# travelingspaceman/LowThrustOpt

Hardware: NVIDIA B200
Metric: segment-propagations/s (fp64 state+STM) (higher is better)
Workload: dtype f64

## Files before the change

lowthrustopt_b200/csrc/lto_capi.cu:

```cuda
#include "../../include/lto_b200.h"
#include "lto_internal.h"
#include "lto_handle.h"
#include <cstdio>
#include <cstring>
#include <cstdarg>
#include <algorithm>
#include <cstdlib>
#include <cmath>
#include <thread>
#include <vector>

using namespace lto;

static char g_err[512] = "";

int lto_fail(lto_handle* h, int code, const char* fmt, ...) {
    char buf[512];
    va_list ap; va_start(ap, fmt); vsnprintf(buf, sizeof buf, fmt, ap); va_end(ap);
    snprintf(g_err, sizeof g_err, "%s", buf);
    if (h) snprintf(h->err, sizeof h->err, "%s", buf);
    return code;
}

int lto_ensure(lto_handle* h, void** p, size_t* cap, size_t need) {
// ... 134 lines not shown
}
double lto_last_kernel_ms(const lto_handle* h) {
    if (!h) return 0.0;
    double ms = h->last_ms;
    for (int i = 0; i < h->n_child; ++i) ms = std::max(ms, h->child[i]->last_ms);
    return ms;
}
int lto_n_devices(const lto_handle* h) { return h ? (h->n_child > 0 ? h->n_child : 1) : 0; }
void* lto_stream(lto_handle* h) { return (h && h->n_child == 0) ? (void*)h->s_compute : nullptr; }
int lto_sync(lto_handle* h) {
    LTO_NVTX();
    if (!h) return fail(nullptr, LTO_ERR_ARG, "null handle");
    for (int i = 0; i < h->n_child; ++i) { int rc = lto_sync(h->child[i]); if (rc) return fail(h, rc, "%s", h->child[i]->err); }
    if (h->n_child > 0) return LTO_SUCCESS;
    CK(h, cudaSetDevice(h->device));
    CK(h, cudaStreamSynchronize(h->s_compute));
    return LTO_SUCCESS;
}

}

static int make_direct(lto_handle* h, const lto_direct_params* p, int nstate, int nsteps, DirectArgs* a) {
    if (!p) return fail(h, LTO_ERR_ARG, "null params");
    if (nstate != 6 && nstate != 7) return fail(h, LTO_ERR_ARG, "nstate must be 6 or 7 (got %d)", nstate);
    if (p->mode != LTO_FIXED && p->mode != LTO_ADAPTIVE) return fail(h, LTO_ERR_ARG, "bad mode %d", p->mode);
    if (p->mode == LTO_FIXED && nsteps < 2) return fail(h, LTO_ERR_ARG, "nsteps must be >= 2 (got %d)", nsteps);
    const double g0 = p->g0 > 0 ? p->g0 : 9.81;
    a->c.mu = p->MU; a->c.m1 = 1.0 - p->MU;
    a->c.kthr = p->TU * p->TU / p->DU / 1e3;
    a->c.cmdot = p->TU / (p->Isp * g0);
    a->c.default_mass = p->default_mass > 0 ? p->default_mass : 1000.0;
    a->cfg.mode = p->mode; a->cfg.nsteps = nsteps; a->cfg.tol = p->tol > 0 ? p->tol : 1e-13;
    a->cfg.err_norm = p->err_norm; a->cfg.max_attempts = p->max_attempts > 0 ? p->max_attempts : 100000;
    return 0;
}
static int make_indirect(lto_handle* h, const lto_indirect_params* p, int ndim, bool sens, IndirectArgs* a) {
    if (!p) return fail(h, LTO_ERR_ARG, "null params");
    if (ndim != 12 && ndim != 14) return fail(h, LTO_ERR_ARG, "ndim must be 12 or 14 (got %d)", ndim);
    if (!(p->p == 0.0 || p->p >= 1.0)) return fail(h, LTO_ERR_ARG, "Invalid value of p!");
    const double g0 = p->g0 > 0 ? p->g0 : 9.81;
    a->c.mu = p->MU; a->c.m1 = 1.0 - p->MU;
    a->c.kthr = p->TU * p->TU / p->DU / 1e3;
    a->c.thrustLimit = p->thrustLimit; a->c.mass = p->mass; a->c.omega = p->time_direction;
    a->c.p = p->p; a->c.rho = p->rho;
    a->c.cm = p->TU / (a->c.kthr * (p->Isp > 0 ? p->Isp : 2000.0) * g0);
    a->cfg.atol = p->abstol > 0 ? p->abstol : 1e-13; a->cfg.rtol = p->reltol > 0 ? p->reltol : 1e-13;
    a->cfg.controller = p->controller; a->cfg.err_norm = sens ? p->err_norm : 0;
    a->cfg.max_attempts = p->max_attempts > 0 ? p->max_attempts : 100000;
    return 0;
}

static int dispatch_direct(lto_handle* h, const DirectArgs& a, int nstate, int kernel) {
    int nl = 0;
    cudaError_t e = cudaErrorNotSupported;
    if (kernel != LTO_KERNEL_GENERIC) e = launch_direct_fast(a, nstate, h->s_compute, &nl);
    if (e == cudaErrorNotSupported) {
        if (kernel == LTO_KERNEL_FAST) return fail(h, LTO_ERR_ARG, "LTO_KERNEL_FAST does not cover this configuration");
        e = launch_direct_generic(a, nstate, h->s_compute, &nl);
    }
    h->launches += nl;
    if (e != cudaSuccess) return fail(h, LTO_ERR_CUDA, "direct kernel launch: %s", cudaGetErrorString(e));
    return 0;
}
static int dispatch_indirect(lto_handle* h, const IndirectArgs& a, int ndim, int kernel, cudaStream_t st = nullptr) {
    int nl = 0;
    if (!st) st = h->s_compute;
// ... 538 lines not shown
```

lowthrustopt_b200/csrc/lto_direct_cw.cu:

```cuda
#include "lto_internal.h"
#include "lto_cw_common.cuh"
#include <algorithm>

namespace lto {

namespace cw {

constexpr int NTILE = 2;
constexpr int NSLOT = 2;
constexpr int XW0 = 2;

template <int NS>
struct Cfg {
    static constexpr int NCOL = NS + 3;
    static constexpr int NW = NTILE + NCOL;
    static constexpr int NTHREADS = 32 * NW;
    static constexpr int SVAL = (NS == 7) ? 10 : 6;
    static constexpr int OFF_H = 13 * SVAL;
    static constexpr int OFF_BM = OFF_H + 1;
    static constexpr int STEP_DOUBLES = OFF_BM + ((NS == 7) ? 3 : 0);
    static constexpr size_t REC_BYTES = (size_t)NTILE * NSLOT * STEP_DOUBLES * 32 * sizeof(double);
    static constexpr int NV = 2 * (NS + 3);
    static constexpr size_t OUT_TILE_BYTES = (size_t)16 * NS * NV * sizeof(double);
    static constexpr size_t OUT_BYTES = (size_t)NTILE * OUT_TILE_BYTES;
    static constexpr size_t BAR_OFF = REC_BYTES + OUT_BYTES;
    static constexpr size_t FLAG_OFF = BAR_OFF + (size_t)NTILE * NSLOT * 2 * sizeof(unsigned long long);
    static constexpr size_t SMEM = FLAG_OFF + (size_t)NTILE * NSLOT * sizeof(int);
};

using namespace cwc;

template <int NS, bool PUB = true>
__device__ __forceinline__ double x_step(double (&r)[3], double (&v)[3], double& m, const double (&u)[3], double omega,
                                         double mdot, double h, const EPConst& c, double* __restrict__ rec, double& maxErr) {
    constexpr int SVAL = Cfg<NS>::SVAL;
    const double h2 = h * h;
    const double w2 = 2.0 * omega;
    const double kom6 = c.kthr / c.default_mass;
    double a[13][3];
    double ev[3] = {0.0, 0.0, 0.0}, ea[3] = {0.0, 0.0, 0.0};
    if (PUB) rec[Cfg<NS>::OFF_H * 32] = h;
#pragma unroll
    for (int j = 0; j < 13; ++j) {
        double R[3], V[3];
#pragma unroll
        for (int q = 0; q < 3; ++q) {
            double accv = 0.0, accr = 0.0;
#pragma unroll
            for (int l = 0; l < j; ++l) {
                if (lto_tab::Bf(j, l) != 0.0) accv = fma(lto_tab::Bf(j, l), a[l][q], accv);
                if (lto_tab::Gf(j, l) != 0.0) accr = fma(lto_tab::Gf(j, l), a[l][q], accr);
            }
            V[q] = (j == 0) ? v[q] : fma(h, accv, v[q]);
            R[q] = (j == 0) ? r[q] : fma(h2, accr, fma(h * lto_tab::Cf(j), v[q], r[q]));
        }
        const double dx1 = R[0] + c.mu, dx2 = dx1 - 1.0;
        const double yz = fma(R[1], R[1], R[2] * R[2]);
        const double i1 = fast_rsqrt(fma(dx1, dx1, yz));
        const double i2 = fast_rsqrt(fma(dx2, dx2, yz));
        const double i1s = i1 * i1, i2s = i2 * i2;
        const double a31 = c.m1 * i1s * i1, a32 = c.mu * i2s * i2;
        const double gg1 = 1.0 - (a31 + a32);
        double kom = kom6, im = 0.0;
        if (NS == 7) { im = fast_rcp(fma(h * lto_tab::Cf(j), mdot, m)); kom = c.kthr * im; }
        a[j][0] = fma(u[0], kom, fma(-a31, dx1, fma(-a32, dx2, fma(w2, V[1], R[0]))));
        a[j][1] = fma(u[1], kom, fma(gg1, R[1], -w2 * V[0]));
        a[j][2] = fma(u[2], kom, (gg1 - 1.0) * R[2]);
        if (PUB && j != 10) {
            const double a51 = 3.0 * i1s * a31, a52 = 3.0 * i2s * a32;
            const double s5 = a51 + a52;
            const double p1 = a51 * dx1, p2 = a52 * dx2;
            const double t = p1 + p2;
            const double s5y = s5 * R[1];
            double* w = rec + j * SVAL * 32;
            w[0 * 32] = fma(p1, dx1, fma(p2, dx2, gg1));
            w[1 * 32] = fma(s5y, R[1], gg1);
            w[2 * 32] = fma(s5 * R[2], R[2], gg1 - 1.0);
            w[3 * 32] = t * R[1];
            w[4 * 32] = t * R[2];
            w[5 * 32] = s5y * R[2];
            if (NS == 7) {
                w[6 * 32] = kom;
                const double k2 = -kom * im;
#pragma unroll
                for (int q = 0; q < 3; ++q) w[(7 + q) * 32] = k2 * u[q];
            }
        }
        if (lto_tab::PSIf(j) != 0.0) {
#pragma unroll
            for (int q = 0; q < 3; ++q) { ev[q] = fma(lto_tab::PSIf(j), V[q], ev[q]); ea[q] = fma(lto_tab::PSIf(j), a[j][q], ea[q]); }
        }
    }
    double delta = 0.0;
#pragma unroll
    for (int q = 0; q < 3; ++q) {
        double sv = 0.0, sr = 0.0;
#pragma unroll
        for (int l = 0; l < 13; ++l) {
            if (lto_tab::CHIf(l) != 0.0) sv = fma(lto_tab::CHIf(l), a[l][q], sv);
            if (lto_tab::CHIBf(l) != 0.0) sr = fma(lto_tab::CHIBf(l), a[l][q], sr);
        }
        r[q] = fma(h2, sr, fma(h, v[q], r[q]));
        v[q] = fma(h, sv, v[q]);
        delta = fmax(delta, fmax(fabs(ev[q]), fabs(ea[q])));
    }
    if (NS == 7) m = fma(h, mdot, m);
    delta *= fabs(h * lto_tab::ERRC);
    maxErr = fmax(maxErr, delta);
    return delta;
}

template <int NS>
__device__ __forceinline__ void col_step(double (&sr)[3], double (&sv)[3], double& sm, double bm, const double (&ec)[3],
                                         double omega, double kom6, const double* __restrict__ rec) {
    constexpr int SVAL = Cfg<NS>::SVAL;
    constexpr bool MASS = (NS == 7);
    const double h = rec[Cfg<NS>::OFF_H * 32];
    const double h2 = h * h;
    const double w2 = 2.0 * omega;
    double a[13][3];
#pragma unroll
    for (int j = 0; j < 13; ++j) {
        if (j == 10) continue;
        double R[3], V[3];
#pragma unroll
        for (int q = 0; q < 3; ++q) {
            double accv = 0.0, accr = 0.0;
#pragma unroll
            for (int l = 0; l < j; ++l) {
                if (lto_tab::Bf(j, l) != 0.0) accv = fma(lto_tab::Bf(j, l), a[l][q], accv);
                if (lto_tab::Gf(j, l) != 0.0) accr = fma(lto_tab::Gf(j, l), a[l][q], accr);
            }
            V[q] = (j == 0) ? sv[q] : fma(h, accv, sv[q]);
            R[q] = (j == 0) ? sr[q] : fma(h2, accr, fma(h * lto_tab::Cf(j), sv[q], sr[q]));
        }
        const double* w = rec + j * SVAL * 32;
        double U[6];
#pragma unroll
        for (int q = 0; q < 6; ++q) U[q] = w[q * 32];
        const double kom = MASS ? w[6 * 32] : kom6;
        double acc[3];
        acc[0] = fma(ec[0], kom, w2 * V[1]);
        acc[1] = fma(ec[1], kom, -w2 * V[0]);
        acc[2] = ec[2] * kom;
        if (MASS) {
            const double smj = fma(h * lto_tab::Cf(j), bm, sm);
#pragma unroll
            for (int q = 0; q < 3; ++q) acc[q] = fma(w[(7 + q) * 32], smj, acc[q]);
        }
        sym3_mul_acc(U, R, acc);
#pragma unroll
        for (int q = 0; q < 3; ++q) a[j][q] = acc[q];
    }
#pragma unroll
    for (int q = 0; q < 3; ++q) {
        double dv = 0.0, dr = 0.0;
#pragma unroll
        for (int l = 0; l < 13; ++l) {
            if (lto_tab::CHIf(l) != 0.0) dv = fma(lto_tab::CHIf(l), a[l][q], dv);
            if (lto_tab::CHIBf(l) != 0.0) dr = fma(lto_tab::CHIBf(l), a[l][q], dr);
        }
        sr[q] = fma(h2, dr, fma(h, sv[q], sr[q]));
        sv[q] = fma(h, dv, sv[q]);
    }
    if (MASS) sm = fma(h, bm, sm);
}

struct ColState { double sr[3], sv[3], sm, bm; };

template <int NS>
__device__ __forceinline__ void col_init(ColState& c, int col) {
#pragma unroll
    for (int q = 0; q < 3; ++q) { c.sr[q] = (col == q) ? 1.0 : 0.0; c.sv[q] = (col == q + 3) ? 1.0 : 0.0; }
    c.sm = (NS == 7 && col == 6) ? 1.0 : 0.0;
    c.bm = 0.0;
}

template <int NS>
__device__ __forceinline__ void col_store(double* __restrict__ stage, const ColState& c, int col, int lane) {
    constexpr int NV = 2 * (NS + 3);
    const int back = lane & 1, gc = col - NS;
    const int ocol = (gc >= 0) ? (2 * NS + (back ? 3 : 0) + gc) : ((back ? NS : 0) + col);
    double* J = stage + (lane >> 1) * (NS * NV) + ocol * NS;
    const double rj = (col >= 3 && col < 6) ? -1.0 : 1.0;
    const double sp = back ? -rj : 1.0;
    const double sq = back ? rj : 1.0;
    J[0] = sp * c.sr[0]; J[1] = sp * c.sr[1]; J[2] = sp * c.sr[2];
    J[3] = sq * c.sv[0]; J[4] = sq * c.sv[1]; J[5] = sq * c.sv[2];
    if (NS == 7) J[6] = sp * c.sm;
}

template <int NS>
__device__ __forceinline__ void column_warp(const DirectArgs& a, long long n_tiles, int col, int lane, double* recs, double* outs, unsigned bars) {
    typedef Cfg<NS> C;
    const int nstep = a.cfg.nsteps - 1;
    const double omega = (lane & 1) ? -1.0 : 1.0;
    const double kom6 = a.c.kthr / a.c.default_mass;
    const int gc = col - NS;
    const double ec[3] = {gc == 0 ? 1.0 : 0.0, gc == 1 ? 1.0 : 0.0, gc == 2 ? 1.0 : 0.0};
    ColState cs[NTILE];
    unsigned g = 0;
    for (long long pair = blockIdx.x; pair * NTILE < n_tiles; pair += gridDim.x) {
#pragma unroll
        for (int t = 0; t < NTILE; ++t) col_init<NS>(cs[t], col);
        for (int k = 0; k < nstep; ++k, ++g) {
            const unsigned slot = g & (NSLOT - 1), par = (g / NSLOT) & 1;
#ifndef LTO_K1_NO_PACE
            asm volatile("bar.sync 3, %0;" ::"n"(32 * C::NCOL) : "memory");
#endif
#pragma unroll
            for (int t = 0; t < NTILE; ++t) {
                const double* rec = recs + (size_t)(t * NSLOT + slot) * C::STEP_DOUBLES * 32 + lane;
                const unsigned full = bars + (unsigned)((t * NSLOT + slot) * 16), empty = full + 8;
                mbar_wait(full, par);
                if (NS == 7 && k == 0 && gc >= 0) cs[t].bm = rec[(C::OFF_BM + gc) * 32];
                col_step<NS>(cs[t].sr, cs[t].sv, cs[t].sm, cs[t].bm, ec, omega, kom6, rec);
                mbar_arrive(empty);
                if (k == nstep - 1) {
                    const long long tile = pair * NTILE + t;
                    const long long seg0 = tile * 16;
                    double* stage = outs + (size_t)t * (C::OUT_TILE_BYTES / sizeof(double));
                    const bool leader = (col == 0 && lane == 0);
                    if (leader) bulk_store_wait_read_but<NTILE - 1>();
                    asm volatile("bar.sync 2, %0;" ::"n"(32 * C::NCOL) : "memory");
                    col_store<NS>(stage, cs[t], col, lane);
                    fence_proxy_async();
                    asm volatile("bar.sync 2, %0;" ::"n"(32 * C::NCOL) : "memory");
                    if (leader && seg0 < a.n_seg) {
                        const long long nseg = (a.n_seg - seg0 < 16) ? (a.n_seg - seg0) : 16;
                        bulk_store(a.jac + seg0 * (long long)(NS * C::NV), smem_u32(stage), (unsigned)(nseg * NS * C::NV * sizeof(double)));
                    }
                }
            }
        }
    }
    if (col == 0 && lane == 0) bulk_store_wait_all();
}

template <int NS>
__device__ __forceinline__ void state_warp(const DirectArgs& a, long long n_tiles, int t, int lane, double* recs, unsigned bars) {
    typedef Cfg<NS> C;
    const int nsteps = a.cfg.nsteps, nstep = nsteps - 1;
    const int back = lane & 1;
    const double omega = back ? -1.0 : 1.0;
    double r[3], v[3], m = a.c.default_mass, u[3], bm[3] = {0.0, 0.0, 0.0}, mdot = 0.0, t0 = 0.0, t1 = 1.0, maxErr = 0.0;
    unsigned g = 0;
    for (long long pair = blockIdx.x; pair * NTILE < n_tiles; pair += gridDim.x) {
        const long long seg = (pair * NTILE + t) * 16 + (lane >> 1);
        {
            const long long sc = seg < a.n_seg ? seg : a.n_seg - 1;
            const long long ia = lto_node_a(sc, a.npt);
            const double* X = (back ? a.Xb : a.Xa) + ia * NS;
            const double* U = (back ? a.ub : a.ua) + ia * 3;
            r[0] = X[0]; r[1] = X[1]; r[2] = X[2];
            v[0] = X[3]; v[1] = X[4]; v[2] = X[5];
            if (back) { v[0] = -v[0]; v[1] = -v[1]; v[2] = -v[2]; }
            if (NS == 7) m = X[6];
            u[0] = U[0]; u[1] = U[1]; u[2] = U[2];
            const double ta = a.ta[ia], tb = a.tb[ia];
            t0 = ta; t1 = ta + (tb - ta) / 2.0;
            const double un = sqrt(fma(u[0], u[0], fma(u[1], u[1], u[2] * u[2])));
            mdot = -omega * un * a.c.cmdot;
            if (NS == 7) {
#pragma unroll
                for (int q = 0; q < 3; ++q) {
                    const double uh = (un > 0.0) ? u[q] / un : 1.0;
                    bm[q] = -omega * a.c.cmdot * uh;
                }
            }
            maxErr = 0.0;
        }
        for (int k = 0; k < nstep; ++k, ++g) {
            const unsigned slot = g & (NSLOT - 1), use = g / NSLOT;
            double* rec = recs + (size_t)(t * NSLOT + slot) * C::STEP_DOUBLES * 32 + lane;
            const unsigned full = bars + (unsigned)((t * NSLOT + slot) * 16), empty = full + 8;
            if (use > 0) mbar_wait(empty, (use - 1) & 1);
            const double h = linrange_at(t0, t1, nsteps, k + 1) - linrange_at(t0, t1, nsteps, k);
            if (NS == 7) {
#pragma unroll
                for (int q = 0; q < 3; ++q) rec[(C::OFF_BM + q) * 32] = bm[q];
            }
            x_step<NS>(r, v, m, u, omega, mdot, h, a.c, rec, maxErr);
            mbar_arrive(full);
        }
        const unsigned fullmask = 0xffffffffu;
        double xe[NS];
        xe[0] = r[0]; xe[1] = r[1]; xe[2] = r[2];
        xe[3] = back ? -v[0] : v[0]; xe[4] = back ? -v[1] : v[1]; xe[5] = back ? -v[2] : v[2];
        if (NS == 7) xe[6] = m;
        bool bad = false;
#pragma unroll
        for (int q = 0; q < NS; ++q) {
            const double other = __shfl_xor_sync(fullmask, xe[q], 1);
            const double d = xe[q] - other;
            bad |= !(d == d);
            if (!back && seg < a.n_seg) a.defect[seg * NS + q] = d;
        }
        const double me_o = __shfl_xor_sync(fullmask, maxErr, 1);
        if (!back && seg < a.n_seg) {
            if (a.errors) a.errors[seg] = fmax(maxErr, me_o);
            if (a.status) a.status[seg] = bad ? LTO_ST_NAN : LTO_OK;
        }
    }
}


template <int NS>
__device__ __forceinline__ void state_warp_adapt(const DirectArgs& a, long long n_tiles, int t, int lane, double* recs, unsigned bars, volatile int* lastf) {
    typedef Cfg<NS> C;
    const int back = lane & 1;
    const double omega = back ? -1.0 : 1.0;
    const unsigned fullmask = 0xffffffffu;
    double r[3], v[3], m = a.c.default_mass, u[3], bm[3] = {0.0, 0.0, 0.0}, mdot = 0.0, dummy = 0.0;
    unsigned g = 0;
    for (long long pair = blockIdx.x; pair * NTILE < n_tiles; pair += gridDim.x) {
        const long long seg = (pair * NTILE + t) * 16 + (lane >> 1);
        const long long sc = seg < a.n_seg ? seg : a.n_seg - 1;
        const long long ia = lto_node_a(sc, a.npt);
        const double* X = (back ? a.Xb : a.Xa) + ia * NS;
        const double* U = (back ? a.ub : a.ua) + ia * 3;
        r[0] = X[0]; r[1] = X[1]; r[2] = X[2];
        v[0] = X[3]; v[1] = X[4]; v[2] = X[5];
        if (back) { v[0] = -v[0]; v[1] = -v[1]; v[2] = -v[2]; }
        if (NS == 7) m = X[6];
        u[0] = U[0]; u[1] = U[1]; u[2] = U[2];
        const double ta = a.ta[ia], tb = a.tb[ia];
        const double t0 = ta, tfinal = ta + (tb - ta) / 2.0;
        const double un = sqrt(fma(u[0], u[0], fma(u[1], u[1], u[2] * u[2])));
        mdot = -omega * un * a.c.cmdot;
        if (NS == 7) {
#pragma unroll
            for (int q = 0; q < 3; ++q) { const double uh = (un > 0.0) ? u[q] / un : 1.0; bm[q] = -omega * a.c.cmdot * uh; }
        }
        const double hmax = (tfinal - t0) / 2.5, hmin = (tfinal - t0) / 1e7;
        double tt = t0, h = (tfinal - t0) / 50.0;
        int status = 0, nt = 0;
        bool done = !((tt < tfinal) && (h >= hmin));
        while (true) {
            const unsigned slot = g & (NSLOT - 1), use = g / NSLOT;
            double* rec = recs + (size_t)(t * NSLOT + slot) * C::STEP_DOUBLES * 32 + lane;
            const unsigned full = bars + (unsigned)((t * NSLOT + slot) * 16), empty = full + 8;
            if (use > 0) mbar_wait(empty, (use - 1) & 1);
            if (NS == 7) {
#pragma unroll
                for (int q = 0; q < 3; ++q) rec[(C::OFF_BM + q) * 32] = bm[q];
            }
            bool pending = !done;
            if (done) {
#pragma unroll
                for (int j = 0; j < 13 * C::SVAL; ++j) rec[j * 32] = 0.0;
                rec[C::OFF_H * 32] = 0.0;
            }
            while (__any_sync(fullmask, pending)) {
                if (pending) {
                    if (tt + h > tfinal) h = tfinal - tt;
                    if (nt >= a.cfg.max_attempts) { status = LTO_ST_MAXSTEPS; done = true; pending = false; }
                }
                if (pending) {
                    ++nt;
                    double r2[3] = {r[0], r[1], r[2]}, v2[3] = {v[0], v[1], v[2]}, m2 = m;
                    const double xn = fmax(fmax(fmax(fabs(r[0]), fabs(r[1])), fmax(fabs(r[2]), fabs(v[0]))), fmax(fmax(fabs(v[1]), fabs(v[2])), NS == 7 ? fabs(m) : 0.0));
                    double delta = x_step<NS>(r2, v2, m2, u, omega, mdot, h, a.c, rec, dummy);
                    if (!(delta == delta)) { status = LTO_ST_NAN; done = true; pending = false; }
                    else {
                        const double tau = a.cfg.tol * fmax(xn, 1.0);
                        if (delta <= tau) {
                            tt += h;
                            r[0] = r2[0]; r[1] = r2[1]; r[2] = r2[2]; v[0] = v2[0]; v[1] = v2[1]; v[2] = v2[2]; m = m2;
                            pending = false;
                        }
                        if (delta == 0.0) delta = 1e-16;
                        h = fmin(hmax, 0.8 * h * pow(tau / delta, 0.125));
                        if (!((tt < tfinal) && (h >= hmin))) { done = true; if (pending) { status = LTO_ST_HMIN; pending = false; } }
                    }
                }
            }
            if (status != 0) {
#pragma unroll
                for (int j = 0; j < 13 * C::SVAL; ++j) rec[j * 32] = 0.0;
                rec[C::OFF_H * 32] = 0.0;
            }
            const bool all_done = __all_sync(fullmask, done);
            if (lane == 0) lastf[t * NSLOT + slot] = all_done ? 1 : 0;
            mbar_arrive(full);
            ++g;
            if (all_done) break;
        }
        if (status == 0 && tt < tfinal) status = LTO_ST_HMIN;
        double xe[NS];
        xe[0] = r[0]; xe[1] = r[1]; xe[2] = r[2];
        xe[3] = back ? -v[0] : v[0]; xe[4] = back ? -v[1] : v[1]; xe[5] = back ? -v[2] : v[2];
        if (NS == 7) xe[6] = m;
        bool bad = false;
#pragma unroll
        for (int q = 0; q < NS; ++q) {
            const double other = __shfl_xor_sync(fullmask, xe[q], 1);
            const double d = xe[q] - other;
            bad |= !(d == d);
            if (!back && seg < a.n_seg) a.defect[seg * NS + q] = d;
        }
        const int st_o = __shfl_xor_sync(fullmask, status, 1);
        if (!back && seg < a.n_seg) {
            if (a.errors) a.errors[seg] = 0.0;
            if (a.status) a.status[seg] = status ? status : (st_o ? st_o : (bad ? LTO_ST_NAN : LTO_OK));
        }
    }
}

template <int NS>
__device__ __forceinline__ void column_warp_adapt(const DirectArgs& a, long long n_tiles, int col, int lane, double* recs, double* outs, unsigned bars,
                                                  volatile int* lastf) {
    typedef Cfg<NS> C;
    const double omega = (lane & 1) ? -1.0 : 1.0;
    const double kom6 = a.c.kthr / a.c.default_mass;
    const int gc = col - NS;
    const double ec[3] = {gc == 0 ? 1.0 : 0.0, gc == 1 ? 1.0 : 0.0, gc == 2 ? 1.0 : 0.0};
    ColState cs[NTILE];
    unsigned g[NTILE];
#pragma unroll
    for (int t = 0; t < NTILE; ++t) g[t] = 0;
    for (long long pair = blockIdx.x; pair * NTILE < n_tiles; pair += gridDim.x) {
#pragma unroll
        for (int t = 0; t < NTILE; ++t) col_init<NS>(cs[t], col);
        unsigned alive = (1u << NTILE) - 1u, first = alive;
        while (alive) {
#ifndef LTO_K1_NO_PACE
            asm volatile("bar.sync 3, %0;" ::"n"(32 * C::NCOL) : "memory");
#endif
#pragma unroll
            for (int t = 0; t < NTILE; ++t) {
                if (!(alive & (1u << t))) continue;
                const unsigned slot = g[t] & (NSLOT - 1), par = (g[t] / NSLOT) & 1;
                const double* rec = recs + (size_t)(t * NSLOT + slot) * C::STEP_DOUBLES * 32 + lane;
                const unsigned full = bars + (unsigned)((t * NSLOT + slot) * 16), empty = full + 8;
                mbar_wait(full, par);
                if (NS == 7 && (first & (1u << t)) && gc >= 0) cs[t].bm = rec[(C::OFF_BM + gc) * 32];
                first &= ~(1u << t);
                const bool last = lastf[t * NSLOT + slot] != 0;
                col_step<NS>(cs[t].sr, cs[t].sv, cs[t].sm, cs[t].bm, ec, omega, kom6, rec);
                mbar_arrive(empty);
                ++g[t];
                if (last) alive &= ~(1u << t);
            }
        }
#pragma unroll
        for (int t = 0; t < NTILE; ++t) {
            const long long tile = pair * NTILE + t;
            const long long seg0 = tile * 16;
            double* stage = outs + (size_t)t * (C::OUT_TILE_BYTES / sizeof(double));
            const bool leader = (col == 0 && lane == 0);
            if (leader) bulk_store_wait_read_but<NTILE - 1>();
            asm volatile("bar.sync 2, %0;" ::"n"(32 * C::NCOL) : "memory");
            col_store<NS>(stage, cs[t], col, lane);
            fence_proxy_async();
            asm volatile("bar.sync 2, %0;" ::"n"(32 * C::NCOL) : "memory");
            if (leader && seg0 < a.n_seg) {
                const long long nseg = (a.n_seg - seg0 < 16) ? (a.n_seg - seg0) : 16;
                bulk_store(a.jac + seg0 * (long long)(NS * C::NV), smem_u32(stage), (unsigned)(nseg * NS * C::NV * sizeof(double)));
            }
        }
    }
    if (col == 0 && lane == 0) bulk_store_wait_all();
}

template <int NS, bool ADAPT>
__global__ void __launch_bounds__(Cfg<NS>::NTHREADS, 1) k_direct_cw(DirectArgs a, long long n_tiles) {
    typedef Cfg<NS> C;
    extern __shared__ __align__(16) unsigned char smem_raw[];
    double* recs = reinterpret_cast<double*>(smem_raw);
    double* outs = reinterpret_cast<double*>(smem_raw + C::REC_BYTES);
    const unsigned bars = smem_u32(smem_raw + C::BAR_OFF);
    const int warp = threadIdx.x >> 5, lane = threadIdx.x & 31;
    if (threadIdx.x == 0) {
#pragma unroll
        for (int i = 0; i < NTILE * NSLOT; ++i) {
            mbar_init(bars + i * 16, 32);
            mbar_init(bars + i * 16 + 8, 32 * C::NCOL);
        }
    }
    __syncthreads();
    volatile int* lastf = reinterpret_cast<volatile int*>(smem_raw + C::FLAG_OFF);
    if (warp >= XW0 && warp < XW0 + NTILE) {
        if (ADAPT) state_warp_adapt<NS>(a, n_tiles, warp - XW0, lane, recs, bars, lastf);
        else state_warp<NS>(a, n_tiles, warp - XW0, lane, recs, bars);
    } else {
        const int col = warp < XW0 ? warp : warp - NTILE;
        if (ADAPT) column_warp_adapt<NS>(a, n_tiles, col, lane, recs, outs, bars, lastf);
        else column_warp<NS>(a, n_tiles, col, lane, recs, outs, bars);
    }
}

template <int NS>
__global__ void __launch_bounds__(128) k_direct_state(DirectArgs a) {
    const int nsteps = a.cfg.nsteps, nstep = nsteps - 1;
    const int lane = threadIdx.x & 31, back = lane & 1;
    const double omega = back ? -1.0 : 1.0;
    const long long n_pairs32 = (a.n_seg + 15) / 16;
    const long long warp0 = ((long long)blockIdx.x * blockDim.x + threadIdx.x) >> 5, nwarp = ((long long)gridDim.x * blockDim.x) >> 5;
    for (long long w = warp0; w < n_pairs32; w += nwarp) {
        const long long seg = w * 16 + (lane >> 1);
        const long long sc = seg < a.n_seg ? seg : a.n_seg - 1;
        const long long ia = lto_node_a(sc, a.npt);
        const double* X = (back ? a.Xb : a.Xa) + ia * NS;
        const double* U = (back ? a.ub : a.ua) + ia * 3;
        double r[3] = {X[0], X[1], X[2]}, v[3] = {X[3], X[4], X[5]}, m = a.c.default_mass, u[3] = {U[0], U[1], U[2]}, maxErr = 0.0;
        if (back) { v[0] = -v[0]; v[1] = -v[1]; v[2] = -v[2]; }
        if (NS == 7) m = X[6];
        const double ta = a.ta[ia], tb = a.tb[ia];
        const double t0 = ta, t1 = ta + (tb - ta) / 2.0;
        const double un = sqrt(fma(u[0], u[0], fma(u[1], u[1], u[2] * u[2])));
        const double mdot = -omega * un * a.c.cmdot;
        for (int k = 0; k < nstep; ++k) {
            const double h = linrange_at(t0, t1, nsteps, k + 1) - linrange_at(t0, t1, nsteps, k);
            x_step<NS, false>(r, v, m, u, omega, mdot, h, a.c, nullptr, maxErr);
        }
        const unsigned fullmask = 0xffffffffu;
        double xe[NS];
        xe[0] = r[0]; xe[1] = r[1]; xe[2] = r[2];
        xe[3] = back ? -v[0] : v[0]; xe[4] = back ? -v[1] : v[1]; xe[5] = back ? -v[2] : v[2];
        if (NS == 7) xe[6] = m;
        bool bad = false;
#pragma unroll
        for (int q = 0; q < NS; ++q) {
            const double other = __shfl_xor_sync(fullmask, xe[q], 1);
            const double d = xe[q] - other;
            bad |= !(d == d);
            if (!back && seg < a.n_seg) a.defect[seg * NS + q] = d;
        }
        const double me_o = __shfl_xor_sync(fullmask, maxErr, 1);
        if (!back && seg < a.n_seg) {
            if (a.errors) a.errors[seg] = fmax(maxErr, me_o);
            if (a.status) a.status[seg] = bad ? LTO_ST_NAN : LTO_OK;
        }
    }
}

}

template <int NS>
static cudaError_t launch_state(const DirectArgs& a, cudaStream_t st) {
    int dev = 0, n_sm = 0;
    cudaError_t e = cudaGetDevice(&dev); if (e != cudaSuccess) return e;
    e = cudaDeviceGetAttribute(&n_sm, cudaDevAttrMultiProcessorCount, dev); if (e != cudaSuccess) return e;
    const long long n_warps = (a.n_seg + 15) / 16;
    const long long blocks = (n_warps + 3) / 4;
    const int grid = (int)std::min<long long>(blocks, (long long)n_sm * 16);
    cw::k_direct_state<NS><<<grid, 128, 0, st>>>(a);
// ... 48 lines not shown
```

lowthrustopt_b200/csrc/lto_internal.h:

```cpp
#pragma once
#include <cuda_runtime.h>
#include <stdint.h>
#include "lto_prop_generic.cuh"

namespace lto {

struct DirectArgs {
    const double *Xa, *Xb, *ua, *ub, *ta, *tb;
    double *defect, *errors, *jac;
    int32_t* status;
    long long n_seg;
    int npt;
    DirectCfg cfg;
    EPConst c;
};

struct IndirectArgs {
    const double *x0, *t0, *t1, *x_target;
    const double *thrustLimit_arr, *rho_arr;
    double *defect, *phi;
    int32_t *status, *nsteps_out;
    unsigned long long* counter;
    double* scratch;
    unsigned long long* prof;
    long long n_seg;
    int npt;
    IndirectCfg cfg;
    SCConst c;
};

__host__ __device__ inline long long lto_node_a(long long s, int npt) { return npt > 0 ? s + s / (npt - 1) : s; }
__host__ __device__ inline long long lto_traj_of(long long s, int npt) { return npt > 0 ? s / (npt - 1) : s; }

cudaError_t launch_direct_generic(const DirectArgs& a, int nstate, cudaStream_t st, int* n_launch);
cudaError_t launch_indirect_generic(const IndirectArgs& a, int ndim, cudaStream_t st, int* n_launch);
cudaError_t launch_direct_fast(const DirectArgs& a, int nstate, cudaStream_t st, int* n_launch);
cudaError_t launch_indirect_fast(const IndirectArgs& a, int ndim, cudaStream_t st, int* n_launch);
size_t indirect_cw_scratch_bytes(int n_sm);
cudaError_t launch_sumsq_rows(const double* v, long long n_rows, long long len, double* out, cudaStream_t st);
cudaError_t launch_fp64_probe(int iters, double* d_sink, int n_sm, cudaStream_t st, long long* n_threads, int* chains);

}
```

lowthrustopt_b200/csrc/lto_tableau.h:

```cpp
#pragma once
#if defined(__CUDACC__)
#define LTO_TAB_FN __host__ __device__ __forceinline__ constexpr
#else
#define LTO_TAB_FN inline constexpr
#endif
namespace lto_tab {
#define LTO_TAB_C_INIT {0.0, 0.07407407407407407, 0.1111111111111111, 0.16666666666666666, 0.4166666666666667, 0.5, 0.8333333333333334, 0.16666666666666666, 0.6666666666666666, 0.3333333333333333, 1.0, 0.0, 1.0}
static constexpr double C[13] = LTO_TAB_C_INIT;
#if defined(__CUDA_ARCH__)
LTO_TAB_FN double Cf(int i) { constexpr double t[13] = LTO_TAB_C_INIT; return t[i]; }
#else
LTO_TAB_FN double Cf(int i) { return C[i]; }
#endif
#define LTO_TAB_B_INIT { \
    {0.0, 0.0, 0.0, 0.0, 0.0, 0.0, 0.0, 0.0, 0.0, 0.0, 0.0, 0.0, 0.0}, \
    {0.07407407407407407, 0.0, 0.0, 0.0, 0.0, 0.0, 0.0, 0.0, 0.0, 0.0, 0.0, 0.0, 0.0}, \
    {0.027777777777777776, 0.08333333333333333, 0.0, 0.0, 0.0, 0.0, 0.0, 0.0, 0.0, 0.0, 0.0, 0.0, 0.0}, \
    {0.041666666666666664, 0.0, 0.125, 0.0, 0.0, 0.0, 0.0, 0.0, 0.0, 0.0, 0.0, 0.0, 0.0}, \
    {0.4166666666666667, 0.0, -1.5625, 1.5625, 0.0, 0.0, 0.0, 0.0, 0.0, 0.0, 0.0, 0.0, 0.0}, \
    {0.05, 0.0, 0.0, 0.25, 0.2, 0.0, 0.0, 0.0, 0.0, 0.0, 0.0, 0.0, 0.0}, \
    {-0.23148148148148148, 0.0, 0.0, 1.1574074074074074, -2.4074074074074074, 2.314814814814815, 0.0, 0.0, 0.0, 0.0, 0.0, 0.0, 0.0}, \
    {0.10333333333333333, 0.0, 0.0, 0.0, 0.27111111111111114, -0.2222222222222222, 0.014444444444444444, 0.0, 0.0, 0.0, 0.0, 0.0, 0.0}, \
    {2.0, 0.0, 0.0, -8.833333333333334, 15.644444444444444, -11.88888888888889, 0.7444444444444445, 3.0, 0.0, 0.0, 0.0, 0.0, 0.0}, \
    {-0.8425925925925926, 0.0, 0.0, 0.21296296296296297, -7.229629629629629, 5.7592592592592595, -0.31666666666666665, 2.8333333333333335, -0.08333333333333333, 0.0, 0.0, 0.0, 0.0}, \
// ... 27 lines not shown
    {0.006172839506172839, 0.0, 0.0, 0.0, 0.0, 0.0, 0.0, 0.0, 0.0, 0.0, 0.0, 0.0, 0.0}, \
    {0.003472222222222222, 0.010416666666666666, 0.0, 0.0, 0.0, 0.0, 0.0, 0.0, 0.0, 0.0, 0.0, 0.0, 0.0}, \
    {0.021701388888888888, -0.13020833333333334, 0.1953125, 0.0, 0.0, 0.0, 0.0, 0.0, 0.0, 0.0, 0.0, 0.0, 0.0}, \
    {0.09375, 0.0, -0.28125, 0.3125, 0.0, 0.0, 0.0, 0.0, 0.0, 0.0, 0.0, 0.0, 0.0}, \
    {-0.8391203703703703, 0.0, 3.90625, -3.1828703703703702, 0.46296296296296297, 0.0, 0.0, 0.0, 0.0, 0.0, 0.0, 0.0, 0.0}, \
    {0.0985082304526749, 0.0, -0.4236111111111111, 0.38477366255144035, -0.07921810699588477, 0.03343621399176955, 0.0, 0.0, 0.0, 0.0, 0.0, 0.0, 0.0}, \
    {5.69369341563786, 0.0, -25.54861111111111, 22.333847736625515, -3.356625514403292, 1.0565843621399178, 0.043333333333333335, 0.0, 0.0, 0.0, 0.0, 0.0, 0.0}, \
    {-2.516095679012346, 0.0, 11.322916666666666, -9.486882716049383, 1.378641975308642, -0.37191358024691357, -0.021111111111111112, -0.25, 0.0, 0.0, 0.0, 0.0, 0.0}, \
    {1.6726117886178862, 0.0, -7.1135670731707314, 4.207825203252033, -0.7191056910569106, 0.3485772357723577, 0.07317073170731707, 2.067073170731707, -0.036585365853658534, 0.0, 0.0, 0.0, 0.0}, \
    {0.011544715447154472, 0.0, 0.0, -0.6686991869918699, 0.07284552845528455, -0.044715447154471545, 0.007073170731707317, 0.6341463414634146, -0.012195121951219513, 0.0, 0.0, 0.0, 0.0}, \
    {1.6757012195121952, 0.0, -7.1135670731707314, 4.876524390243903, -0.7919512195121952, 0.24695121951219512, 0.05146341463414634, 1.3597560975609757, 0.04878048780487805, 0.14634146341463414, 0.0, 0.0, 0.0}, \
}
static constexpr double G[13][13] = LTO_TAB_G_INIT;
#if defined(__CUDA_ARCH__)
LTO_TAB_FN double Gf(int j, int i) { constexpr double t[13][13] = LTO_TAB_G_INIT; return t[j][i]; }
#else
LTO_TAB_FN double Gf(int j, int i) { return G[j][i]; }
#endif
#define LTO_TAB_CHIB_INIT {0.0, 0.0, 0.0, 0.0, 0.0, 0.1619047619047619, 0.04285714285714286, 0.21428571428571427, 0.010714285714285714, 0.02142857142857143, 0.0, 0.04880952380952381, 0.0}
static constexpr double CHIB[13] = LTO_TAB_CHIB_INIT;
#if defined(__CUDA_ARCH__)
LTO_TAB_FN double CHIBf(int i) { constexpr double t[13] = LTO_TAB_CHIB_INIT; return t[i]; }
#else
LTO_TAB_FN double CHIBf(int i) { return CHIB[i]; }
#endif
#define LTO_TAB_PSIB_INIT {1.0, 0.0, 0.0, 0.0, 0.0, 0.0, 0.0, 0.0, 0.0, 0.0, 0.0, -1.0, 0.0}
static constexpr double PSIB[13] = LTO_TAB_PSIB_INIT;
#if defined(__CUDA_ARCH__)
LTO_TAB_FN double PSIBf(int i) { constexpr double t[13] = LTO_TAB_PSIB_INIT; return t[i]; }
#else
LTO_TAB_FN double PSIBf(int i) { return PSIB[i]; }
#endif
static constexpr double ERRC = 0.04880952380952381;
}
```

Measured before the change: 96.15 million.

## Load RK tableau from constant memory, pack stage records as double2, spread state warps

Tableau coefficients in the fixed-step state and column warps now come from a __constant__ array instead of immediates embedded in each FMA, which shrinks the instruction stream and may ease instruction-cache pressure. Per-stage Jacobian records are written and read as double2 pairs to halve shared-memory transactions. State warps are interleaved among column warps with a stride of four rather than sitting next to each other. Optional clock64 profiling hooks are added behind a macro. The constant-memory loads add per-use latency, and the packed layout assumes SVAL is even.

```diff
diff --git a/lowthrustopt_b200/csrc/lto_capi.cu b/lowthrustopt_b200/csrc/lto_capi.cu
--- a/lowthrustopt_b200/csrc/lto_capi.cu
+++ b/lowthrustopt_b200/csrc/lto_capi.cu
@@ -190,6 +190,7 @@
     a->c.default_mass = p->default_mass > 0 ? p->default_mass : 1000.0;
     a->cfg.mode = p->mode; a->cfg.nsteps = nsteps; a->cfg.tol = p->tol > 0 ? p->tol : 1e-13;
     a->cfg.err_norm = p->err_norm; a->cfg.max_attempts = p->max_attempts > 0 ? p->max_attempts : 100000;
+    a->prof = h->d_prof;
     return 0;
 }
 static int make_indirect(lto_handle* h, const lto_indirect_params* p, int ndim, bool sens, IndirectArgs* a) {
diff --git a/lowthrustopt_b200/csrc/lto_direct_cw.cu b/lowthrustopt_b200/csrc/lto_direct_cw.cu
--- a/lowthrustopt_b200/csrc/lto_direct_cw.cu
+++ b/lowthrustopt_b200/csrc/lto_direct_cw.cu
@@ -9,6 +9,13 @@
 constexpr int NTILE = 2;
 constexpr int NSLOT = 2;
 constexpr int XW0 = 2;
+constexpr int XWS = 4;
+__device__ __forceinline__ int state_tile_of(int warp) {
+    return (warp >= XW0 && (warp - XW0) % XWS == 0 && (warp - XW0) / XWS < NTILE) ? (warp - XW0) / XWS : -1;
+}
+__device__ __forceinline__ int col_of(int warp) {
+    return warp - (warp > XW0 ? min(NTILE, (warp - XW0 - 1) / XWS + 1) : 0);
+}
 
 template <int NS>
 struct Cfg {
@@ -30,10 +37,43 @@
 
 using namespace cwc;
 
-template <int NS, bool PUB = true>
+__constant__ __align__(16) double tab_dev[LTO_TAB_DEV_N] = LTO_TAB_DEV_INIT;
+template <bool CT> __device__ __forceinline__ double tab(int o, double v) { return (CT && o >= 0) ? tab_dev[o] : v; }
+template <bool CT> __device__ __forceinline__ double Bd(int j, int l) { return tab<CT>(lto_tab::Bo(j, l), lto_tab::Bf(j, l)); }
+template <bool CT> __device__ __forceinline__ double Gd(int j, int l) { return tab<CT>(lto_tab::Go(j, l), lto_tab::Gf(j, l)); }
+template <bool CT> __device__ __forceinline__ double Cd(int j) { return tab<CT>(lto_tab::Co(j), lto_tab::Cf(j)); }
+template <bool CT> __device__ __forceinline__ double CHId(int l) { return tab<CT>(lto_tab::CHIo(l), lto_tab::CHIf(l)); }
+template <bool CT> __device__ __forceinline__ double CHIBd(int l) { return tab<CT>(lto_tab::CHIBo(l), lto_tab::CHIBf(l)); }
+
+struct K1Prof {
+#ifdef LTO_K1_PROF
+    long long c[4] = {0, 0, 0, 0}, n = 0, t0 = 0, t = 0;
+    __device__ __forceinline__ void start() { t0 = t = clock64(); }
+    __device__ __forceinline__ void add(int i) { const long long x = clock64(); c[i] += x - t; t = x; }
+    __device__ __forceinline__ void step() { ++n; }
+    __device__ __forceinline__ void flush(const DirectArgs& a, int nw, int lane) {
+        if (a.prof && lane == 0) {
+            unsigned long long* o = a.prof + ((size_t)blockIdx.x * nw + (threadIdx.x >> 5)) * 6;
+            o[0] = c[0]; o[1] = c[1]; o[2] = c[2]; o[3] = c[3]; o[4] = clock64() - t0; o[5] = n;
+        }
+    }
+#else
+    __device__ __forceinline__ void start() {}
+    __device__ __forceinline__ void add(int) {}
+    __device__ __forceinline__ void step() {}
+    __device__ __forceinline__ void flush(const DirectArgs&, int, int) {}
+#endif
+};
+enum { PROF_BODY = 0, PROF_WAIT = 1, PROF_PACE = 2, PROF_STAGE = 3 };
+
+template <int NS, class P, class D>
+__device__ __forceinline__ P* stage_pairs(D* rec, int j, int lane) {
+    return reinterpret_cast<P*>(rec - lane + j * Cfg<NS>::SVAL * 32) + lane;
+}
+
+template <int NS, bool PUB, bool CT>
 __device__ __forceinline__ double x_step(double (&r)[3], double (&v)[3], double& m, const double (&u)[3], double omega,
-                                         double mdot, double h, const EPConst& c, double* __restrict__ rec, double& maxErr) {
-    constexpr int SVAL = Cfg<NS>::SVAL;
+                                         double mdot, double h, const EPConst& c, double* __restrict__ rec, int lane, double& maxErr) {
     const double h2 = h * h;
     const double w2 = 2.0 * omega;
     const double kom6 = c.kthr / c.default_mass;
@@ -48,11 +88,11 @@
             double accv = 0.0, accr = 0.0;
 #pragma unroll
             for (int l = 0; l < j; ++l) {
-                if (lto_tab::Bf(j, l) != 0.0) accv = fma(lto_tab::Bf(j, l), a[l][q], accv);
-                if (lto_tab::Gf(j, l) != 0.0) accr = fma(lto_tab::Gf(j, l), a[l][q], accr);
+                if (lto_tab::Bf(j, l) != 0.0) accv = fma(Bd<CT>(j, l), a[l][q], accv);
+                if (lto_tab::Gf(j, l) != 0.0) accr = fma(Gd<CT>(j, l), a[l][q], accr);
             }
             V[q] = (j == 0) ? v[q] : fma(h, accv, v[q]);
-            R[q] = (j == 0) ? r[q] : fma(h2, accr, fma(h * lto_tab::Cf(j), v[q], r[q]));
+            R[q] = (j == 0) ? r[q] : fma(h2, accr, fma(h * Cd<CT>(j), v[q], r[q]));
         }
         const double dx1 = R[0] + c.mu, dx2 = dx1 - 1.0;
         const double yz = fma(R[1], R[1], R[2] * R[2]);
@@ -62,7 +102,7 @@
         const double a31 = c.m1 * i1s * i1, a32 = c.mu * i2s * i2;
         const double gg1 = 1.0 - (a31 + a32);
         double kom = kom6, im = 0.0;
-        if (NS == 7) { im = fast_rcp(fma(h * lto_tab::Cf(j), mdot, m)); kom = c.kthr * im; }
+        if (NS == 7) { im = fast_rcp(fma(h * Cd<CT>(j), mdot, m)); kom = c.kthr * im; }
         a[j][0] = fma(u[0], kom, fma(-a31, dx1, fma(-a32, dx2, fma(w2, V[1], R[0]))));
         a[j][1] = fma(u[1], kom, fma(gg1, R[1], -w2 * V[0]));
         a[j][2] = fma(u[2], kom, (gg1 - 1.0) * R[2]);
@@ -72,18 +112,14 @@
             const double p1 = a51 * dx1, p2 = a52 * dx2;
             const double t = p1 + p2;
             const double s5y = s5 * R[1];
-            double* w = rec + j * SVAL * 32;
-            w[0 * 32] = fma(p1, dx1, fma(p2, dx2, gg1));
-            w[1 * 32] = fma(s5y, R[1], gg1);
-            w[2 * 32] = fma(s5 * R[2], R[2], gg1 - 1.0);
-            w[3 * 32] = t * R[1];
-            w[4 * 32] = t * R[2];
-            w[5 * 32] = s5y * R[2];
+            double2* w = stage_pairs<NS, double2>(rec, j, lane);
+            w[0 * 32] = make_double2(fma(p1, dx1, fma(p2, dx2, gg1)), fma(s5y, R[1], gg1));
+            w[1 * 32] = make_double2(fma(s5 * R[2], R[2], gg1 - 1.0), t * R[1]);
+            w[2 * 32] = make_double2(t * R[2], s5y * R[2]);
             if (NS == 7) {
-                w[6 * 32] = kom;
                 const double k2 = -kom * im;
-#pragma unroll
-                for (int q = 0; q < 3; ++q) w[(7 + q) * 32] = k2 * u[q];
+                w[3 * 32] = make_double2(kom, k2 * u[0]);
+                w[4 * 32] = make_double2(k2 * u[1], k2 * u[2]);
             }
         }
         if (lto_tab::PSIf(j) != 0.0) {
@@ -97,23 +133,22 @@
         double sv = 0.0, sr = 0.0;
 #pragma unroll
         for (int l = 0; l < 13; ++l) {
-            if (lto_tab::CHIf(l) != 0.0) sv = fma(lto_tab::CHIf(l), a[l][q], sv);
-            if (lto_tab::CHIBf(l) != 0.0) sr = fma(lto_tab::CHIBf(l), a[l][q], sr);
+            if (lto_tab::CHIf(l) != 0.0) sv = fma(CHId<CT>(l), a[l][q], sv);
+            if (lto_tab::CHIBf(l) != 0.0) sr = fma(CHIBd<CT>(l), a[l][q], sr);
         }
         r[q] = fma(h2, sr, fma(h, v[q], r[q]));
         v[q] = fma(h, sv, v[q]);
         delta = fmax(delta, fmax(fabs(ev[q]), fabs(ea[q])));
     }
     if (NS == 7) m = fma(h, mdot, m);
-    delta *= fabs(h * lto_tab::ERRC);
+    delta *= fabs(h * tab<CT>(lto_tab::ERRCo, lto_tab::ERRC));
     maxErr = fmax(maxErr, delta);
     return delta;
 }
 
-template <int NS>
+template <int NS, bool CT>
 __device__ __forceinline__ void col_step(double (&sr)[3], double (&sv)[3], double& sm, double bm, const double (&ec)[3],
-                                         double omega, double kom6, const double* __restrict__ rec) {
-    constexpr int SVAL = Cfg<NS>::SVAL;
+                                         double omega, double kom6, const double* __restrict__ rec, int lane) {
     constexpr bool MASS = (NS == 7);
     const double h = rec[Cfg<NS>::OFF_H * 32];
     const double h2 = h * h;
@@ -128,25 +163,27 @@
             double accv = 0.0, accr = 0.0;
 #pragma unroll
             for (int l = 0; l < j; ++l) {
-                if (lto_tab::Bf(j, l) != 0.0) accv = fma(lto_tab::Bf(j, l), a[l][q], accv);
-                if (lto_tab::Gf(j, l) != 0.0) accr = fma(lto_tab::Gf(j, l), a[l][q], accr);
+                if (lto_tab::Bf(j, l) != 0.0) accv = fma(Bd<CT>(j, l), a[l][q], accv);
+                if (lto_tab::Gf(j, l) != 0.0) accr = fma(Gd<CT>(j, l), a[l][q], accr);
             }
             V[q] = (j == 0) ? sv[q] : fma(h, accv, sv[q]);
-            R[q] = (j == 0) ? sr[q] : fma(h2, accr, fma(h * lto_tab::Cf(j), sv[q], sr[q]));
-        }
-        const double* w = rec + j * SVAL * 32;
-        double U[6];
-#pragma unroll
-        for (int q = 0; q < 6; ++q) U[q] = w[q * 32];
-        const double kom = MASS ? w[6 * 32] : kom6;
+            R[q] = (j == 0) ? sr[q] : fma(h2, accr, fma(h * Cd<CT>(j), sv[q], sr[q]));
+        }
+        const double2* w = stage_pairs<NS, const double2>(rec, j, lane);
+        const double2 p0 = w[0 * 32], p1 = w[1 * 32], p2 = w[2 * 32];
+        const double U[6] = {p0.x, p0.y, p1.x, p1.y, p2.x, p2.y};
+        double2 p3 = make_double2(kom6, 0.0), p4 = make_double2(0.0, 0.0);
+        if (MASS) { p3 = w[3 * 32]; p4 = w[4 * 32]; }
+        const double kom = p3.x;
+        const double am[3] = {p3.y, p4.x, p4.y};
         double acc[3];
         acc[0] = fma(ec[0], kom, w2 * V[1]);
         acc[1] = fma(ec[1], kom, -w2 * V[0]);
         acc[2] = ec[2] * kom;
         if (MASS) {
-            const double smj = fma(h * lto_tab::Cf(j), bm, sm);
-#pragma unroll
-            for (int q = 0; q < 3; ++q) acc[q] = fma(w[(7 + q) * 32], smj, acc[q]);
+            const double smj = fma(h * Cd<CT>(j), bm, sm);
+#pragma unroll
+            for (int q = 0; q < 3; ++q) acc[q] = fma(am[q], smj, acc[q]);
         }
         sym3_mul_acc(U, R, acc);
 #pragma unroll
@@ -157,8 +194,8 @@
         double dv = 0.0, dr = 0.0;
 #pragma unroll
         for (int l = 0; l < 13; ++l) {
-            if (lto_tab::CHIf(l) != 0.0) dv = fma(lto_tab::CHIf(l), a[l][q], dv);
-            if (lto_tab::CHIBf(l) != 0.0) dr = fma(lto_tab::CHIBf(l), a[l][q], dr);
+            if (lto_tab::CHIf(l) != 0.0) dv = fma(CHId<CT>(l), a[l][q], dv);
+            if (lto_tab::CHIBf(l) != 0.0) dr = fma(CHIBd<CT>(l), a[l][q], dr);
         }
         sr[q] = fma(h2, dr, fma(h, sv[q], sr[q]));
         sv[q] = fma(h, dv, sv[q]);
@@ -200,6 +237,8 @@
     const double ec[3] = {gc == 0 ? 1.0 : 0.0, gc == 1 ? 1.0 : 0.0, gc == 2 ? 1.0 : 0.0};
     ColState cs[NTILE];
     unsigned g = 0;
+    K1Prof prof;
+    prof.start();
     for (long long pair = blockIdx.x; pair * NTILE < n_tiles; pair += gridDim.x) {
 #pragma unroll
         for (int t = 0; t < NTILE; ++t) col_init<NS>(cs[t], col);
@@ -208,14 +247,18 @@
 #ifndef LTO_K1_NO_PACE
             asm volatile("bar.sync 3, %0;" ::"n"(32 * C::NCOL) : "memory");
 #endif
+            prof.add(PROF_PACE);
 #pragma unroll
             for (int t = 0; t < NTILE; ++t) {
                 const double* rec = recs + (size_t)(t * NSLOT + slot) * C::STEP_DOUBLES * 32 + lane;
                 const unsigned full = bars + (unsigned)((t * NSLOT + slot) * 16), empty = full + 8;
                 mbar_wait(full, par);
+                prof.add(PROF_WAIT);
                 if (NS == 7 && k == 0 && gc >= 0) cs[t].bm = rec[(C::OFF_BM + gc) * 32];
-                col_step<NS>(cs[t].sr, cs[t].sv, cs[t].sm, cs[t].bm, ec, omega, kom6, rec);
+                col_step<NS, true>(cs[t].sr, cs[t].sv, cs[t].sm, cs[t].bm, ec, omega, kom6, rec, lane);
                 mbar_arrive(empty);
+                prof.add(PROF_BODY);
+                prof.step();
                 if (k == nstep - 1) {
                     const long long tile = pair * NTILE + t;
                     const long long seg0 = tile * 16;
@@ -230,11 +273,13 @@
                         const long long nseg = (a.n_seg - seg0 < 16) ? (a.n_seg - seg0) : 16;
                         bulk_store(a.jac + seg0 * (long long)(NS * C::NV), smem_u32(stage), (unsigned)(nseg * NS * C::NV * sizeof(double)));
                     }
+                    prof.add(PROF_STAGE);
                 }
             }
         }
     }
     if (col == 0 && lane == 0) bulk_store_wait_all();
+    prof.flush(a, C::NW, lane);
 }
 
 template <int NS>
@@ -245,6 +290,8 @@
     const double omega = back ? -1.0 : 1.0;
     double r[3], v[3], m = a.c.default_mass, u[3], bm[3] = {0.0, 0.0, 0.0}, mdot = 0.0, t0 = 0.0, t1 = 1.0, maxErr = 0.0;
     unsigned g = 0;
+    K1Prof prof;
+    prof.start();
     for (long long pair = blockIdx.x; pair * NTILE < n_tiles; pair += gridDim.x) {
         const long long seg = (pair * NTILE + t) * 16 + (lane >> 1);
         {
@@ -270,18 +317,22 @@
             }
             maxErr = 0.0;
         }
+        prof.add(PROF_STAGE);
         for (int k = 0; k < nstep; ++k, ++g) {
             const unsigned slot = g & (NSLOT - 1), use = g / NSLOT;
             double* rec = recs + (size_t)(t * NSLOT + slot) * C::STEP_DOUBLES * 32 + lane;
             const unsigned full = bars + (unsigned)((t * NSLOT + slot) * 16), empty = full + 8;
             if (use > 0) mbar_wait(empty, (use - 1) & 1);
+            prof.add(PROF_WAIT);
             const double h = linrange_at(t0, t1, nsteps, k + 1) - linrange_at(t0, t1, nsteps, k);
             if (NS == 7) {
 #pragma unroll
                 for (int q = 0; q < 3; ++q) rec[(C::OFF_BM + q) * 32] = bm[q];
             }
-            x_step<NS>(r, v, m, u, omega, mdot, h, a.c, rec, maxErr);
+            x_step<NS, true, true>(r, v, m, u, omega, mdot, h, a.c, rec, lane, maxErr);
             mbar_arrive(full);
+            prof.add(PROF_BODY);
+            prof.step();
         }
         const unsigned fullmask = 0xffffffffu;
         double xe[NS];
@@ -301,7 +352,9 @@
             if (a.errors) a.errors[seg] = fmax(maxErr, me_o);
             if (a.status) a.status[seg] = bad ? LTO_ST_NAN : LTO_OK;
         }
-    }
+        prof.add(PROF_STAGE);
+    }
+    prof.flush(a, C::NW, lane);
 }
 
 
@@ -347,8 +400,9 @@
             }
             bool pending = !done;
             if (done) {
-#pragma unroll
-                for (int j = 0; j < 13 * C::SVAL; ++j) rec[j * 32] = 0.0;
+                double2* z = stage_pairs<NS, double2>(rec, 0, lane);
+#pragma unroll
+                for (int p = 0; p < 13 * C::SVAL / 2; ++p) z[p * 32] = make_double2(0.0, 0.0);
                 rec[C::OFF_H * 32] = 0.0;
             }
             while (__any_sync(fullmask, pending)) {
@@ -360,7 +414,7 @@
                     ++nt;
                     double r2[3] = {r[0], r[1], r[2]}, v2[3] = {v[0], v[1], v[2]}, m2 = m;
                     const double xn = fmax(fmax(fmax(fabs(r[0]), fabs(r[1])), fmax(fabs(r[2]), fabs(v[0]))), fmax(fmax(fabs(v[1]), fabs(v[2])), NS == 7 ? fabs(m) : 0.0));
-                    double delta = x_step<NS>(r2, v2, m2, u, omega, mdot, h, a.c, rec, dummy);
+                    double delta = x_step<NS, true, false>(r2, v2, m2, u, omega, mdot, h, a.c, rec, lane, dummy);
                     if (!(delta == delta)) { status = LTO_ST_NAN; done = true; pending = false; }
                     else {
                         const double tau = a.cfg.tol * fmax(xn, 1.0);
@@ -376,8 +430,9 @@
                 }
             }
             if (status != 0) {
-#pragma unroll
-                for (int j = 0; j < 13 * C::SVAL; ++j) rec[j * 32] = 0.0;
+                double2* z = stage_pairs<NS, double2>(rec, 0, lane);
+#pragma unroll
+                for (int p = 0; p < 13 * C::SVAL / 2; ++p) z[p * 32] = make_double2(0.0, 0.0);
                 rec[C::OFF_H * 32] = 0.0;
             }
             const bool all_done = __all_sync(fullmask, done);
@@ -437,7 +492,7 @@
                 if (NS == 7 && (first & (1u << t)) && gc >= 0) cs[t].bm = rec[(C::OFF_BM + gc) * 32];
                 first &= ~(1u << t);
                 const bool last = lastf[t * NSLOT + slot] != 0;
-                col_step<NS>(cs[t].sr, cs[t].sv, cs[t].sm, cs[t].bm, ec, omega, kom6, rec);
+                col_step<NS, false>(cs[t].sr, cs[t].sv, cs[t].sm, cs[t].bm, ec, omega, kom6, rec, lane);
                 mbar_arrive(empty);
                 ++g[t];
                 if (last) alive &= ~(1u << t);
@@ -480,11 +535,12 @@
     }
     __syncthreads();
     volatile int* lastf = reinterpret_cast<volatile int*>(smem_raw + C::FLAG_OFF);
-    if (warp >= XW0 && warp < XW0 + NTILE) {
-        if (ADAPT) state_warp_adapt<NS>(a, n_tiles, warp - XW0, lane, recs, bars, lastf);
-        else state_warp<NS>(a, n_tiles, warp - XW0, lane, recs, bars);
+    const int st = state_tile_of(warp);
+    if (st >= 0) {
+        if (ADAPT) state_warp_adapt<NS>(a, n_tiles, st, lane, recs, bars, lastf);
+        else state_warp<NS>(a, n_tiles, st, lane, recs, bars);
     } else {
-        const int col = warp < XW0 ? warp : warp - NTILE;
+        const int col = col_of(warp);
         if (ADAPT) column_warp_adapt<NS>(a, n_tiles, col, lane, recs, outs, bars, lastf);
         else column_warp<NS>(a, n_tiles, col, lane, recs, outs, bars);
     }
@@ -512,7 +568,7 @@
         const double mdot = -omega * un * a.c.cmdot;
         for (int k = 0; k < nstep; ++k) {
             const double h = linrange_at(t0, t1, nsteps, k + 1) - linrange_at(t0, t1, nsteps, k);
-            x_step<NS, false>(r, v, m, u, omega, mdot, h, a.c, nullptr, maxErr);
+            x_step<NS, false, false>(r, v, m, u, omega, mdot, h, a.c, nullptr, lane, maxErr);
         }
         const unsigned fullmask = 0xffffffffu;
         double xe[NS];
diff --git a/lowthrustopt_b200/csrc/lto_internal.h b/lowthrustopt_b200/csrc/lto_internal.h
--- a/lowthrustopt_b200/csrc/lto_internal.h
+++ b/lowthrustopt_b200/csrc/lto_internal.h
@@ -9,6 +9,7 @@
     const double *Xa, *Xb, *ua, *ub, *ta, *tb;
     double *defect, *errors, *jac;
     int32_t* status;
+    unsigned long long* prof;
     long long n_seg;
     int npt;
     DirectCfg cfg;
diff --git a/lowthrustopt_b200/csrc/lto_tableau.h b/lowthrustopt_b200/csrc/lto_tableau.h
--- a/lowthrustopt_b200/csrc/lto_tableau.h
+++ b/lowthrustopt_b200/csrc/lto_tableau.h
@@ -83,4 +83,45 @@
 LTO_TAB_FN double PSIBf(int i) { return PSIB[i]; }
 #endif
 static constexpr double ERRC = 0.04880952380952381;
+#define LTO_TAB_DEV_N 124
+#define LTO_TAB_DEV_INIT {0.07407407407407407, 0.07407407407407407, 0.027777777777777776, 0.006172839506172839, 0.08333333333333333, 0.1111111111111111, 0.041666666666666664, 0.003472222222222222, 0.010416666666666666, 0.16666666666666666, 0.4166666666666667, 0.021701388888888888, -0.13020833333333334, 0.4166666666666667, 0.05, 0.2, -0.23148148148148148, -0.8391203703703703, 1.1574074074074074, -3.1828703703703702, -2.4074074074074074, 0.46296296296296297, 2.314814814814815, 0.8333333333333334, 0.10333333333333333, 0.0985082304526749, -0.4236111111111111, 0.38477366255144035, 0.27111111111111114, -0.07921810699588477, -0.2222222222222222, 0.03343621399176955, 0.014444444444444444, 0.16666666666666666, 5.69369341563786, -25.54861111111111, -8.833333333333334, 22.333847736625515, 15.644444444444444, -3.356625514403292, -11.88888888888889, 1.0565843621399178, 0.7444444444444445, 0.043333333333333335, 0.6666666666666666, 0.0, -0.8425925925925926, -2.516095679012346, 11.322916666666666, 0.21296296296296297, -9.486882716049383, -7.229629629629629, 1.378641975308642, 5.7592592592592595, -0.37191358024691357, -0.31666666666666665, -0.021111111111111112, 2.8333333333333335, -0.08333333333333333, 0.3333333333333333, 0.5812195121951219, 1.6726117886178862, -7.1135670731707314, -2.0792682926829267, 4.207825203252033, 4.3863414634146345, -0.7191056910569106, -3.6707317073170733, 0.3485772357723577, 0.5202439024390244, 0.07317073170731707, 0.5487804878048781, 2.067073170731707, 0.27439024390243905, -0.036585365853658534, 0.43902439024390244, 0.014634146341463415, 0.011544715447154472, -0.6686991869918699, 0.07284552845528455, -0.14634146341463414, -0.044715447154471545, -0.014634146341463415, 0.007073170731707317, -0.07317073170731707, 0.6341463414634146, 0.07317073170731707, -0.012195121951219513, 0.14634146341463414, 0.0, -0.43341463414634146, 1.6757012195121952, -7.1135670731707314, -2.0792682926829267, 4.876524390243903, 4.3863414634146345, -0.7919512195121952, -3.524390243902439, 0.24695121951219512, 0.5348780487804878, 0.05146341463414634, 0.6219512195121951, 1.3597560975609757, 0.20121951219512196, 0.04878048780487805, 0.2926829268292683, 0.14634146341463414, 0.0, 0.3238095238095238, 0.1619047619047619, 0.2571428571428571, 0.04285714285714286, 0.2571428571428571, 0.21428571428571427, 0.03214285714285714, 0.010714285714285714, 0.03214285714285714, 0.02142857142857143, 0.04880952380952381, 0.04880952380952381, 0.04880952380952381, 0.0, 0.04880952380952381, 0.0}
+#define LTO_TAB_C_DEV_INIT {-1, 1, 5, 9, 13, -1, 23, 33, 44, 59, -1, -1, -1}
+LTO_TAB_FN int Co(int i) { constexpr short t[13] = LTO_TAB_C_DEV_INIT; return t[i]; }
+#define LTO_TAB_B_DEV_INIT { \
+    {-1, -1, -1, -1, -1, -1, -1, -1, -1, -1, -1, -1, -1}, \
+    {0, -1, -1, -1, -1, -1, -1, -1, -1, -1, -1, -1, -1}, \
+    {2, 4, -1, -1, -1, -1, -1, -1, -1, -1, -1, -1, -1}, \
+    {6, -1, -1, -1, -1, -1, -1, -1, -1, -1, -1, -1, -1}, \
+    {10, -1, -1, -1, -1, -1, -1, -1, -1, -1, -1, -1, -1}, \
+    {14, -1, -1, -1, 15, -1, -1, -1, -1, -1, -1, -1, -1}, \
+    {16, -1, -1, 18, 20, 22, -1, -1, -1, -1, -1, -1, -1}, \
+    {24, -1, -1, -1, 28, 30, 32, -1, -1, -1, -1, -1, -1}, \
+    {-1, -1, -1, 36, 38, 40, 42, -1, -1, -1, -1, -1, -1}, \
+    {46, -1, -1, 49, 51, 53, 55, 57, 58, -1, -1, -1, -1}, \
+    {60, -1, -1, 63, 65, 67, 69, 71, 73, 75, -1, -1, -1}, \
+    {76, -1, -1, -1, -1, 80, 82, 84, 86, 88, -1, -1, -1}, \
+    {90, -1, -1, 93, 95, 97, 99, 101, 103, 105, -1, -1, -1}, \
 }
+LTO_TAB_FN int Bo(int j, int i) { constexpr short t[13][13] = LTO_TAB_B_DEV_INIT; return t[j][i]; }
+#define LTO_TAB_CHI_DEV_INIT {-1, -1, -1, -1, -1, 108, 110, 112, 114, 116, -1, 118, 120}
+LTO_TAB_FN int CHIo(int i) { constexpr short t[13] = LTO_TAB_CHI_DEV_INIT; return t[i]; }
+#define LTO_TAB_G_DEV_INIT { \
+    {-1, -1, -1, -1, -1, -1, -1, -1, -1, -1, -1, -1, -1}, \
+    {-1, -1, -1, -1, -1, -1, -1, -1, -1, -1, -1, -1, -1}, \
+    {3, -1, -1, -1, -1, -1, -1, -1, -1, -1, -1, -1, -1}, \
+    {7, 8, -1, -1, -1, -1, -1, -1, -1, -1, -1, -1, -1}, \
+    {11, 12, -1, -1, -1, -1, -1, -1, -1, -1, -1, -1, -1}, \
+    {-1, -1, -1, -1, -1, -1, -1, -1, -1, -1, -1, -1, -1}, \
+    {17, -1, -1, 19, 21, -1, -1, -1, -1, -1, -1, -1, -1}, \
+    {25, -1, 26, 27, 29, 31, -1, -1, -1, -1, -1, -1, -1}, \
+    {34, -1, 35, 37, 39, 41, 43, -1, -1, -1, -1, -1, -1}, \
+    {47, -1, 48, 50, 52, 54, 56, -1, -1, -1, -1, -1, -1}, \
+    {61, -1, 62, 64, 66, 68, 70, 72, 74, -1, -1, -1, -1}, \
+    {77, -1, -1, 78, 79, 81, 83, 85, 87, -1, -1, -1, -1}, \
+    {91, -1, 92, 94, 96, 98, 100, 102, 104, 106, -1, -1, -1}, \
+}
+LTO_TAB_FN int Go(int j, int i) { constexpr short t[13][13] = LTO_TAB_G_DEV_INIT; return t[j][i]; }
+#define LTO_TAB_CHIB_DEV_INIT {-1, -1, -1, -1, -1, 109, 111, 113, 115, 117, -1, 119, -1}
+LTO_TAB_FN int CHIBo(int i) { constexpr short t[13] = LTO_TAB_CHIB_DEV_INIT; return t[i]; }
+static constexpr int ERRCo = 122;
+}
```

After: 95.26 million (median of 6 runs). About the same (-0.9%).
